# snap-research/MMVID

Measured on AMD Instinct MI355X. Metric: video-tokens/sec training step, 8-frame 128px text-to-video, higher is better.
Workload: dtype bf16

## Files before the change

### include/mmvid_hip_ext.h

```cpp
#ifndef MMVID_HIP_EXT_H
#define MMVID_HIP_EXT_H
#include <stdint.h>
#ifdef __cplusplus
extern "C" {
#endif

int mmvid_variates_fill(const int64_t* seeds, const int32_t* substream, int64_t videos, int64_t rows_per_video, int64_t n,
                        int purpose, int kind, const int32_t* draw_dev, int64_t draw_first, int64_t draws,
                        float* out, void* stream);

int mmvid_ema_update(float* ema, const float* p, int64_t n, float decay, int warmup, int step, const float* step_dev,
                     const uint8_t* row_flags, int64_t table_lo, int64_t table_rows, int rowlen, void* stream);

int mmvid_step_guard(const float* sqnorm, float grad_scale, float* step_dev, int32_t* guard_i, float* guard_f, void* stream);
int mmvid_adam_step_guarded(float* p, const float* g, float* m, float* v, void* shadow_bf16, int64_t n, float lr, const float* lr_dev,
                            float beta1, float beta2, float eps, float weight_decay, int step, const float* step_dev, float max_norm,
                            const float* sqnorm, float grad_scale, const uint8_t* row_flags, int64_t table_lo, int64_t table_rows,
                            int rowlen, const int32_t* skip_dev, void* stream);
int mmvid_ema_update_guarded(float* ema, const float* p, int64_t n, float decay, int warmup, int step, const float* step_dev,
                             const uint8_t* row_flags, int64_t table_lo, int64_t table_rows, int rowlen, const int32_t* skip_dev,
                             void* stream);

int mmvid_logits_truncate_rows(const float* logits, const float* logits_u, int64_t ld, const float* scale_dev, int64_t rows_per_scale,
                               float logit_div, int top_k, float top_p, const int32_t* top_k_dev, const float* top_p_dev,
// ... 6 lines not shown
                        const uint8_t* row_flags, int64_t table_lo, int64_t table_rows, int rowlen, const int32_t* skip_dev,
                        int32_t every, int32_t slots, int32_t* count_dev, float* partials_f, int32_t* partials_i,
                        float* ring_f, int32_t* ring_i, int32_t* head_i, float* head_f, void* stream);

int mmvid_adam_step_decoupled(float* p, const float* g, float* m, float* v, void* shadow_bf16, int64_t n, float lr, const float* lr_dev,
                              float beta1, float beta2, float eps, float weight_decay, int step, const float* step_dev, float max_norm,
                              const float* sqnorm, float grad_scale, const uint8_t* row_flags, int64_t table_lo, int64_t table_rows,
                              int rowlen, const int32_t* skip_dev, void* stream);

int mmvid_lr_schedule_ext(const float* step_dev, int kind, float lr_min, float lr_max, int every, int64_t a, int64_t b, float gamma,
                          float* lr_out, void* stream);

int mmvid_lr_plateau(const float* loss_dev, const float* step_dev, int every, float factor, int patience, int cooldown, float threshold,
                     float min_lr, float eps, float* state_f, int32_t* state_i, const int32_t* skip_dev, void* stream);

#ifdef __cplusplus
}
#endif
#endif
```

### mmvid_amd/clip_tower.py

```python
import ctypes
import os
import math

import torch
from torch import nn

from . import _lib, ops
from .functional import _note_params, _with_param_zeros
from .shadow import Bf16Weight

TOWER_SHAPES = {
    'openai_clip_visual': (768, 12, 12),
    'openai_clip_text': (512, 12, 8),
}
MAX_WIDTH = 1024
MATRIX_KEYS = ('attn.in_proj_weight', 'attn.out_proj.weight', 'mlp.c_fc.weight', 'mlp.c_proj.weight')


def check_tower_width(width, source):
    if width <= 0 or width % 64:
        raise ValueError(f'{source}: tower width {width} is not a multiple of 64 (the attention kernels take heads of 64: heads = width / 64)')
    if width > MAX_WIDTH:
        raise ValueError(f'{source}: tower width {width} is above {MAX_WIDTH}, the widest tower the kernels take '
                         '(ViT-L/14 visual towers are 1024 wide; ViT-H and larger are not supported)')
# ... 53 lines not shown
        self.resblocks = nn.ModuleList([ResidualAttentionBlockParams(width, layers) for _ in range(layers)])


class _TowerFn(torch.autograd.Function):
    @staticmethod
    def forward(ctx, x, tower, keep, *params):
        _note_params(ctx, (x, tower, keep) + params)
        ctx.tower = tower
        y, saved = tower._run_forward(x, keep=keep)
        ctx.saved_arena = saved
        ctx.shape = x.shape
        return y

    @staticmethod
    def backward(ctx, gy):
        g = gy.contiguous().clone()
        ctx.tower._run_backward(g, ctx.saved_arena, ctx.shape)
        ctx.saved_arena = None
        return _with_param_zeros(ctx, (g.view(ctx.shape), None, None) + (None, ) * (len(ctx.needs_input_grad) - 3))


class DecodeSession:

    def __init__(self, tower, kv_cache, first_pos, graph, fused=True):
        self.tower, self.cache, self.fused = tower, kv_cache, fused
        B, dev = kv_cache.shape[1], kv_cache.device
        self.cfg = tower._cfg(B, kv_cache.shape[2])
        self.layers, self._keep = tower._layer_structs(False)
        _, self.scratch = tower._workspace(self.cfg, dev, False)
        self.x = torch.zeros(B, tower.width, device=dev, dtype=torch.float32)
        self.y = torch.zeros_like(self.x)
        self.pos = torch.tensor([first_pos], dtype=torch.int32, device=dev)
# ... 97 lines not shown
            raise ValueError(f'dim={model_dim} does not match the tower: {source} gives a {which_model} tower {width} wide; pass dim={width}')
        self.width, self.layers, self.heads = width or w, layers or l, heads or h
        self.debug_keep_saved = False
        assert self.width == 64 * self.heads, 'head_dim must be 64 (CLIP towers)'
        self.context_length = seq_len
        self.causal = causal
        self.transformer = _TowerParams(self.width, self.layers)
        self.mask_spec = self.build_attention_mask(seq_len, mask_type, **(mask_kwargs or {})) if causal else None
        if model_path is not None:
            self.load_clip_checkpoint(model_path, which_model, sd)
        self._matrix_holders = [h for blk in self.transformer.resblocks for h in (
            (blk.attn, 'in_proj_weight'), (blk.attn.out_proj, 'weight'), (blk.mlp.c_fc, 'weight'), (blk.mlp.c_proj, 'weight'))]
        self._bf16 = [None] * len(self._matrix_holders)
        self._scratch = None
        self._scratch_retired = []
        self.backward_chunk_layers = int(os.environ.get('MMVID_BWD_CHUNK', 0))
        self.on_layers_done = None

    @staticmethod
    def build_attention_mask(context_length, mask_type='causal', **kwargs):
        if mask_type == 'causal':
            return 'causal'
        if mask_type == 'mask_prev':
            idx = list(kwargs['index'])
            assert len(idx) <= 2, 'the kernels carry at most two restricted rows (BERT uses [ST1],[VID])'
            return ('rows', [(int(i), int(i)) for i in idx])
        raise NotImplementedError(mask_type)

    def dense_attention_mask(self, L=None):
        L = L or self.context_length
# ... 108 lines not shown
            a.g_out_w, a.g_out_b = gptr(blk.attn.out_proj.weight), gptr(blk.attn.out_proj.bias)
            a.g_fc_w, a.g_fc_b = gptr(blk.mlp.c_fc.weight), gptr(blk.mlp.c_fc.bias)
            a.g_pj_w, a.g_pj_b = gptr(blk.mlp.c_proj.weight), gptr(blk.mlp.c_proj.bias)
        return arr, keep

    def _workspace(self, cfg, device, keep):
        sb, cb = ctypes.c_int64(), ctypes.c_int64()
        _lib.call('mmvid_tower_workspace', ctypes.byref(cfg), ctypes.byref(sb), ctypes.byref(cb))
        if self._scratch is None or self._scratch.device != torch.device(device) or self._scratch.numel() < cb.value:
            if self._scratch is not None:
                self._scratch_retired.append(self._scratch)
            self._scratch = torch.empty(cb.value, device=device, dtype=torch.uint8)
        saved = torch.empty(sb.value, device=device, dtype=torch.uint8) if keep else None
        return saved, self._scratch

    def _run_forward(self, x, keep):
        x = ops._chk(x.contiguous(), torch.float32, 'tower input')
        B, L, _ = x.shape
        cfg = self._cfg(B, L)
        layers, _keep = self._layer_structs(False)
        saved, scratch = self._workspace(cfg, x.device, keep)
        y = torch.empty_like(x)
        _lib.call('mmvid_tower_forward', ctypes.byref(cfg), layers, ops._p(x), ops._p(y), ops._p(saved), ops._p(scratch),
                  ops._stream())
        if self.debug_keep_saved:
            self._last_saved = saved
        return y, saved

    def backward_chunks(self):
        if self.on_layers_done is None:
            return [(0, self.layers)]
        if self.backward_chunk_layers <= 0:
            return self._planned_chunks()
        step = self.backward_chunk_layers
        out, hi = [], self.layers
        while hi > 0:
# ... 4 lines not shown

    def _planned_chunks(self):
        if getattr(self, '_chunk_plan', None) is None or self._chunk_plan[0] != self.layers:
            E = self.width
            F = 4 * E
            t = sum(-(-n // 256) * -(-k // 128) for n, k in ((3 * E, E), (E, E), (F, E), (E, F)))
            waste = lambda n: (-(-n * t // 256)) - n * t / 256.0
            best, plan = None, [(0, self.layers)]
            for a in range(3, self.layers - 2):
                w = waste(a) + waste(self.layers - a) + 0.02 * abs(a - 0.6 * self.layers)
                if best is None or w < best:
                    best, plan = w, [(self.layers - a, self.layers), (0, self.layers - a)]
            self._chunk_plan = (self.layers, plan)
        return self._chunk_plan[1]

    def _run_backward(self, g, saved, shape):
        if saved is None:
            raise _lib.MMVIDError('tower backward without saved activations (forward ran under no_grad)')
        B, L, _ = shape
        cfg = self._cfg(B, L)
        layers, _keep = self._layer_structs(True)
        _, scratch = self._workspace(cfg, g.device, False)
        sb = ctypes.c_int64()
        _lib.call('mmvid_tower_workspace', ctypes.byref(cfg), ctypes.byref(sb), None)
        if sb.value != saved.numel():
            raise _lib.MMVIDError(f'tower backward: the saved arena holds {saved.numel()} bytes, the current layout needs {sb.value} '
                                  '(the library changed between forward and backward)')
        per_layer = saved.numel() // self.layers
        for lo, hi in self.backward_chunks():
            sub = self._cfg(B, L)
            sub.layers = hi - lo
            lp = ctypes.cast(ctypes.byref(layers, lo * ctypes.sizeof(_lib.TowerLayer)), ctypes.POINTER(_lib.TowerLayer))
            _lib.call('mmvid_tower_backward', ctypes.byref(sub), lp, ops._p(g),
                      ctypes.c_void_p(saved.data_ptr() + lo * per_layer), ops._p(scratch), ops._stream())
            if self.on_layers_done is not None:
                self.on_layers_done(lo)
```

### mmvid_amd/csrc/embed.hip

```cpp
#include "../../include/mmvid_hip.h"
#include "common.h"

namespace {

constexpr int MAX_TABLES = 4;
struct Tables {
    const float* t[MAX_TABLES];
    long rows[MAX_TABLES];
};
struct GradTables {
    float* t[MAX_TABLES];
    long rows[MAX_TABLES];
};

__device__ unsigned long long g_faults[4];

__global__ __launch_bounds__(256) void assemble_fwd_kernel(Tables tb, const long long* __restrict__ ids,
                                                           const int* __restrict__ seg,
                                                           const float* __restrict__ pos, long nrows, int L, int E,
                                                           float* __restrict__ out) {
    const long row = (long)blockIdx.x * 4 + (threadIdx.x >> 6);
    if (row >= nrows) return;
    const int lane = threadIdx.x & 63;
    const int l = (int)(row % L);
// ... 160 lines not shown
    const float l = lse[row];
    long t = target[row];
    if (t < 0 || t >= V) t = 0;
    const float4* p = reinterpret_cast<const float4*>(logits + row * ldl);
    for (int c = lane; c < (V >> 2); c += 64) {
        const float4 v = p[c];
        float o[4] = {__expf(v.x - l), __expf(v.y - l), __expf(v.z - l), __expf(v.w - l)};
        const long base = (long)c * 4;
#pragma unroll
        for (int e = 0; e < 4; ++e)
            if (base + e == t) o[e] -= 1.0f;
        d[c] = make_uint2(pack_bf2(o[0] * gs, o[1] * gs), pack_bf2(o[2] * gs, o[3] * gs));
    }
}

template <bool DET>
__global__ __launch_bounds__(256) void colsum_bf16_kernel(const bf16_t* __restrict__ dy, long ld, long M, int N,
                                                          float* __restrict__ db) {
    __shared__ float red[8][256];
    const int cc = threadIdx.x & 31, rg = threadIdx.x >> 5;
    const int n = (blockIdx.x * 32 + cc) * 8;
    const long m0 = (long)blockIdx.y * 256;
    float a[8];
#pragma unroll
    for (int e = 0; e < 8; ++e) a[e] = 0.f;
    if (n < N) {
        long m1 = m0 + 256;
        if (m1 > M) m1 = M;
        for (long m = m0 + rg; m < m1; m += 8) {
            const uint4 w = *reinterpret_cast<const uint4*>(dy + m * ld + n);
            a[0] += bf_lo(w.x), a[1] += bf_hi(w.x), a[2] += bf_lo(w.y), a[3] += bf_hi(w.y);
            a[4] += bf_lo(w.z), a[5] += bf_hi(w.z), a[6] += bf_lo(w.w), a[7] += bf_hi(w.w);
        }
    }
#pragma unroll
    for (int e = 0; e < 8; ++e) red[rg][cc * 8 + e] = a[e];
    __syncthreads();
    const int col = threadIdx.x;
    const int gn = blockIdx.x * 256 + col;
    if (gn < N) {
        float s = 0.f;
#pragma unroll
        for (int r = 0; r < 8; ++r) s += red[r][col];
        if (DET)
            db[(long)blockIdx.y * N + gn] = s;
        else
            unsafeAtomicAdd(db + gn, s);
    }
}
// ... 249 lines not shown
                                       const uint8_t* select, const float* lse, const float* gscale, int64_t rows,
                                       int V, void* dlogits_bf16, int64_t ldd, void* stream) {
    MMVID_REQUIRE(logits && target && lse && gscale && dlogits_bf16, "cross_entropy_bwd: null pointer");
    MMVID_REQUIRE(V % 4 == 0 && ldl % 4 == 0 && ldd % 4 == 0, "cross_entropy_bwd: V/ld must be multiples of 4");
    if (rows == 0) return MMVID_OK;
    hipLaunchKernelGGL(ce_bwd_kernel, dim3(cdiv(rows, 4)), dim3(256), 0, (hipStream_t)stream, logits, (long)ldl,
                       (const long long*)target, select, lse, gscale, (long)rows, V, (bf16_t*)dlogits_bf16, (long)ldd);
    MMVID_LAUNCH_CHECK("cross_entropy_bwd");
    return MMVID_OK;
}

extern "C" int mmvid_colsum_bf16(const void* dy, int64_t ld, int64_t M, int N, float* db, void* stream) {
    MMVID_REQUIRE(dy && db, "colsum_bf16: null pointer");
    MMVID_REQUIRE(N % 8 == 0 && ld % 8 == 0, "colsum_bf16: N and ld must be multiples of 8");
    if (M == 0) return MMVID_OK;
    hipLaunchKernelGGL(colsum_bf16_kernel<false>, dim3(cdiv(N, 256), cdiv(M, 256)), dim3(256), 0, (hipStream_t)stream,
                       (const bf16_t*)dy, (long)ld, (long)M, N, db);
    MMVID_LAUNCH_CHECK("colsum_bf16");
    return MMVID_OK;
}

int mmvid_slab_reduce(const float* slab, int nslabs, int N, float* out, hipStream_t stream) {
    hipLaunchKernelGGL(slab_reduce_kernel, dim3(cdiv(N, 32)), dim3(256), 0, stream, slab, nslabs, N, out);
    return MMVID_OK;
}

extern "C" int64_t mmvid_colsum_bf16_det_workspace_bytes(int64_t M, int N) { return (int64_t)cdiv(M > 0 ? M : 1, 256) * N * 4; }

extern "C" int mmvid_colsum_bf16_det(const void* dy, int64_t ld, int64_t M, int N, float* db, void* workspace,
                                     int64_t workspace_bytes, void* stream) {
    MMVID_REQUIRE(dy && db, "colsum_bf16_det: null pointer");
    MMVID_REQUIRE(N % 8 == 0 && ld % 8 == 0, "colsum_bf16_det: N and ld must be multiples of 8");
    if (M == 0) return MMVID_OK;
    MMVID_REQUIRE(workspace && workspace_bytes >= mmvid_colsum_bf16_det_workspace_bytes(M, N),
                  "colsum_bf16_det: workspace of %lld bytes needed (mmvid_colsum_bf16_det_workspace_bytes)",
                  (long long)mmvid_colsum_bf16_det_workspace_bytes(M, N));
    const int blocks = cdiv(M, 256);
    hipLaunchKernelGGL(colsum_bf16_kernel<true>, dim3(cdiv(N, 256), blocks), dim3(256), 0, (hipStream_t)stream, (const bf16_t*)dy,
                       (long)ld, (long)M, N, (float*)workspace);
    mmvid_slab_reduce((const float*)workspace, blocks, N, db, (hipStream_t)stream);
    MMVID_LAUNCH_CHECK("colsum_bf16_det");
    return MMVID_OK;
}

extern "C" int64_t mmvid_cross_entropy_fwd_det_workspace_bytes(int64_t rows) { return (rows > 0 ? rows : 1) * 4; }

extern "C" int mmvid_cross_entropy_fwd_det(const float* logits, int64_t ldl, const int64_t* target, const uint8_t* select,
                                           int64_t rows, int V, float* lse, float* loss_sum, void* workspace,
                                           int64_t workspace_bytes, void* stream) {
    MMVID_REQUIRE(logits && target && lse && loss_sum, "cross_entropy_fwd_det: null pointer");
    MMVID_REQUIRE(V % 4 == 0 && ldl % 4 == 0, "cross_entropy_fwd_det: V and ldl must be multiples of 4");
    if (rows == 0) return MMVID_OK;
    MMVID_REQUIRE(workspace && workspace_bytes >= rows * 4, "cross_entropy_fwd_det: workspace of %lld bytes needed", (long long)rows * 4);
    hipLaunchKernelGGL(ce_fwd_kernel<true>, dim3(cdiv(rows, 4)), dim3(256), 0, (hipStream_t)stream, logits, (long)ldl,
// ... 318 lines not shown
```

### mmvid_amd/csrc/tower.hip

```cpp
#include "../../include/mmvid_hip.h"
#include "common.h"
#include <vector>

#include "graphs.h"

namespace {

inline int64_t align256(int64_t x) { return (x + 255) & ~(int64_t)255; }
constexpr int kMaxSplitK = 16;
constexpr int kLnBwdBlocks = 512;

struct Dims {
    int B, L, E, H, F, layers;
    int64_t M;
};
Dims dims_of(const mmvid_tower_cfg_t& c) {
    Dims d;
    d.B = c.B, d.L = c.L, d.E = c.E, d.H = c.H, d.F = c.F, d.layers = c.layers;
    d.M = (int64_t)c.B * c.L;
    return d;
}

struct SavedLayer {
    int64_t x_in, x_mid, mean1, rstd1, mean2, rstd2, h1, qkv, o, lse2, h2, pre, act, k_gpj, k_dpre, k_gout, k_dqkv, k_ln1, k_ln2, total;
// ... 88 lines not shown
}

}

extern "C" int mmvid_tower_workspace(const mmvid_tower_cfg_t* cfg, int64_t* saved_bytes, int64_t* scratch_bytes) {
    TRY(check_cfg(cfg));
    const Dims d = dims_of(*cfg);
    if (saved_bytes) *saved_bytes = saved_layout(d).total * d.layers;
    if (scratch_bytes) *scratch_bytes = scratch_layout(d).total;
    return MMVID_OK;
}

static int tower_forward_enqueue(const mmvid_tower_cfg_t* cfg, const mmvid_tower_layer_t* layers, const float* x_in,
                                 float* x_out, void* saved, void* scratch, void* stream, void* kv_cache = nullptr,
                                 int kv_lmax = 0);
static int tower_backward_enqueue(const mmvid_tower_cfg_t* cfg, const mmvid_tower_layer_t* layers, float* g,
                                  void* saved, void* scratch, void* stream);

static uint64_t tower_key(uint64_t seed, const mmvid_tower_cfg_t* cfg, const mmvid_tower_layer_t* layers, const void* a,
                          const void* b, const void* c, const void* d, const void* stream) {
    uint64_t k = mmvid_hash_bytes(cfg, sizeof(*cfg), 0xcbf29ce484222325ull ^ seed);
    k = mmvid_hash_bytes(layers, sizeof(mmvid_tower_layer_t) * (size_t)cfg->layers, k);
    return mmvid_hash_ptr(stream, mmvid_hash_ptr(d, mmvid_hash_ptr(c, mmvid_hash_ptr(b, mmvid_hash_ptr(a, k)))));
}

extern "C" int mmvid_tower_forward(const mmvid_tower_cfg_t* cfg, const mmvid_tower_layer_t* layers,
                                   const float* x_in, float* x_out, void* saved, void* scratch, void* stream) {
    TRY(check_cfg(cfg));
    MMVID_REQUIRE(layers && x_in && x_out && scratch, "tower_forward: null pointer");
    const uint64_t key = tower_key(2, cfg, layers, x_in, x_out, saved, scratch, stream);
    return mmvid_run_cached(key, (hipStream_t)stream, [=](hipStream_t s) {
        return tower_forward_enqueue(cfg, layers, x_in, x_out, saved, scratch, (void*)s);
    });
}

static int tower_forward_enqueue(const mmvid_tower_cfg_t* cfg, const mmvid_tower_layer_t* layers, const float* x_in,
                                 float* x_out, void* saved, void* scratch, void* stream, void* kv_cache, int kv_lmax) {
    const Dims d = dims_of(*cfg);
    const SavedLayer sl = saved_layout(d);
    const Scratch sc = scratch_layout(d);
    char* scr = (char*)scratch;
    const float scale = 0.125f;
    const float* x = x_in;
    for (int i = 0; i < d.layers; ++i) {
        const mmvid_tower_layer_t& ly = layers[i];
        char* sv = saved ? (char*)saved + (int64_t)i * sl.total : scr + sc.infer;
        float* xin_s = (float*)(sv + sl.x_in);
        float* xmid = (float*)(sv + sl.x_mid);
        if (saved && i == 0) {
            if (hipMemcpyAsync(xin_s, x_in, d.M * d.E * 4, hipMemcpyDeviceToDevice, (hipStream_t)stream) != hipSuccess) {
                mmvid_set_error("tower_forward: memcpy failed");
                return MMVID_ERR_HIP;
            }
            x = xin_s;
        }
        float* xnext;
        if (i == d.layers - 1)
            xnext = x_out;
        else if (saved)
            xnext = (float*)((char*)saved + (int64_t)(i + 1) * sl.total + sl.x_in);
        else
            xnext = x_out;
        TRY(mmvid_layernorm_fwd(x, d.E, d.M, d.E, ly.ln1_w, ly.ln1_b, cfg->ln_eps, sv + sl.h1, nullptr, d.E,
                                (float*)(sv + sl.mean1), (float*)(sv + sl.rstd1), stream));
        TRY(linear_fwd(d.M, 3 * d.E, d.E, sv + sl.h1, ly.in_w, ly.in_b, nullptr, nullptr, 0, nullptr, sv + sl.qkv, stream));
        if (kv_cache)
            TRY(mmvid_kv_store(sv + sl.qkv, 3 * d.E, d.B, d.L, d.E, nullptr, 0, kv_lmax,
                               (char*)kv_cache + (int64_t)i * d.B * kv_lmax * 2 * d.E * 2, stream));
        TRY(mmvid_attention_fwd(sv + sl.qkv, 3 * d.E, d.B, d.L, d.H, d.E, scale, cfg->mask_mode, cfg->r0, cfg->c0, cfg->r1,
                                cfg->c1, sv + sl.o, d.E, (float*)(sv + sl.lse2), stream));
        TRY(linear_fwd(d.M, d.E, d.E, sv + sl.o, ly.out_w, ly.out_b, x, nullptr, 0, xmid, nullptr, stream));
        TRY(mmvid_layernorm_fwd(xmid, d.E, d.M, d.E, ly.ln2_w, ly.ln2_b, cfg->ln_eps, sv + sl.h2, nullptr, d.E,
                                (float*)(sv + sl.mean2), (float*)(sv + sl.rstd2), stream));
        TRY(linear_fwd(d.M, d.F, d.E, sv + sl.h2, ly.fc_w, ly.fc_b, nullptr, saved ? sv + sl.pre : nullptr, 1, nullptr,
                       sv + sl.act, stream));
        TRY(linear_fwd(d.M, d.E, d.F, sv + sl.act, ly.pj_w, ly.pj_b, xmid, nullptr, 0, xnext, nullptr, stream));
        x = xnext;
    }
    return MMVID_OK;
}

extern "C" int mmvid_tower_backward(const mmvid_tower_cfg_t* cfg, const mmvid_tower_layer_t* layers, float* g,
                                    void* saved, void* scratch, void* stream) {
    TRY(check_cfg(cfg));
    MMVID_REQUIRE(layers && g && saved && scratch, "tower_backward: null pointer");
    const uint64_t key = tower_key(mmvid_option(MMVID_OPT_DETERMINISTIC) ? 5 : 3, cfg, layers, g, saved, scratch, nullptr, stream);
    return mmvid_run_cached(key, (hipStream_t)stream, [=](hipStream_t s) {
        return tower_backward_enqueue(cfg, layers, g, saved, scratch, (void*)s);
    });
}

static int tower_backward_enqueue(const mmvid_tower_cfg_t* cfg, const mmvid_tower_layer_t* layers, float* g, void* saved,
                                  void* scratch, void* stream) {
    const Dims d = dims_of(*cfg);
    const SavedLayer sl = saved_layout(d);
    const Scratch sc = scratch_layout(d);
    char* scr = (char*)scratch;
    char* keep = (char*)saved;
    struct { int64_t g_pj, d_pre, g_out, dqkv, total; } kl = {sl.k_gpj, sl.k_dpre, sl.k_gout, sl.k_dqkv, sl.total};
    const float scale = 0.125f;
    void* d_h = scr + sc.d_h;
    float* ws = (float*)(scr + sc.splitk_ws);
    void* det_ws = nullptr;
    const int64_t det_bytes = det_slab_bytes(d);
    if (mmvid_option(MMVID_OPT_DETERMINISTIC)) {
        MMVID_REQUIRE(det_bytes <= sc.total - sc.infer, "tower_backward: the deterministic slabs do not fit the scratch arena");
        det_ws = scr + sc.infer;
    }
    const int64_t ln_ws_floats = (int64_t)kLnBwdBlocks * 3 * d.E;
    std::vector<mmvid_ln_reduce_t> ln_items;
    int ln_blocks = 0;
    for (int i = d.layers - 1; i >= 0; --i) {
        const mmvid_tower_layer_t& ly = layers[i];
        const char* sv = (const char*)saved + (int64_t)i * sl.total;
        char* kp = keep + (int64_t)i * kl.total;
        void* g_pj = kp + kl.g_pj;
        if (i == d.layers - 1) {
            TRY(mmvid_cast_f32_to_bf16(g, g_pj, d.M * d.E, stream));
            if (ly.g_pj_b && det_ws) TRY(mmvid_colsum_bf16_det(g_pj, d.E, d.M, d.E, ly.g_pj_b, det_ws, det_bytes, stream));
            if (ly.g_pj_b && !det_ws) TRY(mmvid_colsum_bf16(g_pj, d.E, d.M, d.E, ly.g_pj_b, stream));
        }
        TRY(linear_dx(d.M, d.E, d.F, g_pj, ly.pj_w, sv + sl.pre, nullptr, kp + kl.d_pre, stream, ly.g_fc_b, det_ws, det_bytes));
        TRY(linear_dx(d.M, d.F, d.E, kp + kl.d_pre, ly.fc_w, nullptr, nullptr, d_h, stream));
        {
            mmvid_ln_reduce_t r = {(const float*)(kp + sl.k_ln2), ly.g_ln2_w, ly.g_ln2_b, ly.g_out_b};
            int nb = 0;
            TRY(mmvid_layernorm_bwd_partial(d_h, 1, d.E, (const float*)(sv + sl.x_mid), d.E, (const float*)(sv + sl.mean2),
                                            (const float*)(sv + sl.rstd2), ly.ln2_w, d.M, d.E, g, d.E, 1, kp + kl.g_out, r.dw != nullptr,
                                            r.db != nullptr, r.dx_colsum != nullptr, (float*)(kp + sl.k_ln2), ln_ws_floats, &nb, stream));
            if (r.dw || r.db || r.dx_colsum) ln_items.push_back(r), ln_blocks = nb;
        }
        TRY(linear_dx(d.M, d.E, d.E, kp + kl.g_out, ly.out_w, nullptr, nullptr, scr + sc.d_o, stream));
        if (det_ws)
            TRY(mmvid_attention_bwd_bias_det(sv + sl.qkv, 3 * d.E, sv + sl.o, d.E, scr + sc.d_o, d.E, (const float*)(sv + sl.lse2),
                                             (float*)(scr + sc.delta), d.B, d.L, d.H, d.E, scale, cfg->mask_mode, cfg->r0, cfg->c0,
// ... 96 lines not shown
```

### mmvid_amd/dalle_artv.py

```python
import torch
import torch.nn.functional as F
from torch import nn

from . import artv_sampling, ops, sampling, seeded, token_draw
from .artv_sampling import k_keep, keep_top
from .clip_tower import OpenAICLIPTransformer, check_tower_width
from .dalle_bert import DivideMax, eval_decorator, exists, set_requires_grad
from .frontend import Frontend, check_condition_drop, face_choices
from .functional import AssembleSequence, LNLinear, LNLinearCrossEntropy
from .modules import AxialPositionalEmbedding, AxialPositionalEmbeddingList
from .shadow import Bf16Weight

NEG = -torch.finfo(torch.float32).max


def is_empty(t):
    return t.nelement() == 0


def top_k(logits, thres=0.5):
    return keep_top(logits, k_keep(thres, logits.shape[-1]))


class DALLE(nn.Module):
# ... 150 lines not shown
        return text, torch.where(vis_tok == -1, vis_pad, vis_tok)

    def _pos_rows(self):
        return torch.cat([self.text_pos_emb.weight, self.visual_pos_emb.table(), self.image_pos_emb.table()], 0)

    def _hidden(self, text, vis_tok, image):
        text, visual = self._prompt_ids(text, vis_tok)
        parts = [text, visual]
        if exists(image) and not is_empty(image):
            image = self.get_image_tokens(image)
            parts.append(image)
        ids = torch.cat(parts, 1)
        if ids.shape[1] > self.total_seq_len:
            ids = ids[:, :-1]
        L = ids.shape[1]
        x = AssembleSequence.apply(self._pos_rows()[:L], ids.contiguous(), self._seg[:L].contiguous(), self.text_emb.weight,
                                   self.visual_emb.weight, self.image_emb.weight)
        out = self.transformer(x)
        if self.stable:
            out = self.norm_by_max(out)
        return out, text, visual, image

    def _logits_rows(self, rows, cols=None):
        lin = self.to_logits[1]
        if cols is None:
            return LNLinear.apply(rows, self.to_logits[0].weight, self.to_logits[0].bias, lin.weight, lin.bias, self._w16())
        with torch.no_grad():
            hn = ops.layernorm_fwd(rows.contiguous(), self.to_logits[0].weight, self.to_logits[0].bias, 1e-5, save_stats=False)[0]
            return ops.gemm(hn, self._w16()[cols[0]:cols[1]], bias=lin.bias.detach()[cols[0]:cols[1]], out_dtype=torch.float32)

    def forward(self, text, visual=None, target=None, return_loss=False, erase_visual=False, erase_visual_half=False,
# ... 176 lines not shown
```

### mmvid_amd/dalle_bert.py

```python
import torch
import torch.nn.functional as F
from torch import nn

from . import ops, sampling, seeded
from .clip_tower import OpenAICLIPTransformer, check_tower_width
from .frontend import Frontend, check_condition_drop, face_choices
from .functional import PosTable, AssembleSequence, BertHeads, LNLinear, Linear, LayerNormRows
from .shadow import Bf16Weight
from .modules import AxialPositionalEmbedding, AxialPositionalEmbeddingList


def exists(val):
    return val is not None


def set_requires_grad(model, value):
    if model is not None:
        for p in model.parameters():
            p.requires_grad = value


def eval_decorator(fn):
    def inner(model, *args, **kwargs):
        was_training = model.training
# ... 274 lines not shown
        choices, frame0 = face_choices(vc_mode, face_mode)
        return self.frontend.erase_choice(image, tv, f, self.image_token_lut['[MASK]'], choices, frame0)

    def _visual_tokens(self, visual, erase_visual, erase_visual_half, vc_mode, face_mode, visual_aug_mode):
        if self.num_visuals == 0 or not (exists(visual) and len(visual)):
            return None
        if visual_aug_mode == 'motion_color' and torch.is_tensor(visual) and visual.dim() == 5:
            visual = self.frontend.visual_color_jitter(visual, 0.9, 1)
        tok = self.get_image_tokens(visual, insert_sep=self.insert_sep, which_vae='cvae')
        if erase_visual:
            tok = self.random_erase_codebook(tok, self.visual_eraser, erase_visual_half)
        if vc_mode is not None:
            tok = self.erase_codebook_face(tok, vc_mode, face_mode)
        return tok

    def _assemble(self, ids, length, text_rows=None):
        pos = self._pos_table()[:length]
        x = AssembleSequence.apply(pos, ids.contiguous(), self._seg[:length].contiguous(), *self._tables())
        if x.requires_grad:
            x.register_hook(self._note_table_backward)
        if text_rows is not None:
            x[:, self.txt_tok_index].add_(text_rows)
        return x

    def _map_text_feature(self, feat):
        m = self.text_feature_mapping
        if isinstance(m, nn.Linear):
            return Linear.apply(feat, m.weight, m.bias, self._w16(m))
        h = LNLinear.apply(feat, m[0].weight, m[0].bias, m[1].weight, m[1].bias, self._w16(m[1]))
        h = LNLinear.apply(h, m[2].weight, m[2].bias, m[3].weight, m[3].bias, self._w16(m[3]))
        return LayerNormRows.apply(h, m[4].weight, m[4].bias)

    def _head_rows(self, B, nseq, device):
# ... 102 lines not shown
        self.frontend.advance(device)

        if rel:
            assert B >= 2 and B % 2 == 0
        text_neg_ids = None
        if rel and negvc:
            text_neg_ids = ops._chk(text_neg.contiguous(), torch.int64, 'text_neg')
        ids, sel, tfull, cnt = ops.bert_build_ids(text, vis_tok, self.visual_seq_len, target, target_warp, mask1, pad_base, MASK,
                                                  bool(rel), bool(do_vid), text_neg=text_neg_ids)
        self._log_text_ids(ids)
        if text_rows is not None and (rel or do_vid):
            half = B // 2
            per_pass = [text_rows] + ([torch.cat((text_rows[half:], text_rows[:half]))] if rel else []) + \
                ([text_rows] if do_vid else [])
            text_rows = torch.cat(per_pass)
        x_seq = self._assemble(ids, self.total_seq_len, text_rows)
        if text_neg_ids is not None and self.num_visuals > 0 and self.visual_seq_len > 0:
            L = self.total_seq_len
            v0 = 1 + self.text_seq_len
            keep = torch.cat((torch.arange(0, v0, device=device), torch.arange(v0 + self.visual_seq_len, L, device=device)))
            x_neg = x_seq[B:2 * B].index_select(1, keep).contiguous()
            x_main = torch.cat((x_seq[:B], x_seq[2 * B:])) if do_vid else x_seq[:B]
            y_main = self.transformer_forward(x_main.contiguous())
            y_neg = self.transformer_forward(x_neg)
            y_rel = torch.zeros(B, L, y_neg.shape[-1], device=device, dtype=y_neg.dtype).index_copy(1, keep, y_neg)
            y = torch.cat((y_main[:B], y_rel, y_main[B:])) if do_vid else torch.cat((y_main, y_rel))
        else:
            y = self.transformer_forward(x_seq)
        if self._debug_keep is not None:
            self._debug_keep.update(mask1=mask1, nfm=not_fully_masked, target=target, target_warp=target_warp, ids=ids, sel=sel,
                                    tfull=tfull, cnt=cnt, x_seq=x_seq, y=y)
        nseq = 1 + int(bool(rel)) + int(bool(do_vid))
# ... 66 lines not shown
```

### mmvid_amd/functional.py

```python
import torch

from . import ops

bf16, f32 = torch.bfloat16, torch.float32


def _grad_buf(p):
    if p.grad is None:
        p.grad = torch.zeros_like(p)
    return p.grad


_ZERO = {}


def _inside_ddp():
    ddp = getattr(torch.nn.parallel, 'DistributedDataParallel', None)
    return ddp is not None and getattr(ddp, '_active_ddp_module', None) is not None


def _note_params(ctx, args):
    ctx._ddp_params = [a if (isinstance(a, torch.nn.Parameter) and a.requires_grad) else None for a in args] if _inside_ddp() else None


# ... 3 lines not shown
        return grads
    out = list(grads)
    for i, p in enumerate(ps):
        if p is not None and i < len(out) and out[i] is None:
            _grad_buf(p)
            key = (p.device, p.dtype)
            if key not in _ZERO:
                _ZERO[key] = torch.zeros((), device=p.device, dtype=p.dtype)
            out[i] = _ZERO[key].expand(p.shape)
    return tuple(out)


class AssembleSequence(torch.autograd.Function):

    @staticmethod
    def forward(ctx, pos, ids, seg, *tables):
        _note_params(ctx, (pos, ids, seg) + tables)
        ctx.tables = tables
        ctx.save_for_backward(ids, seg)
        return ops.assemble_sequence([t.detach() for t in tables], ids, seg, pos.detach().contiguous())

    @staticmethod
    def backward(ctx, dx):
        ids, seg = ctx.saved_tensors
        dx = dx.contiguous()
        gts = [_grad_buf(t) if t.requires_grad else None for t in ctx.tables]
        dpos = torch.empty(dx.shape[1:], device=dx.device, dtype=f32) if ctx.needs_input_grad[0] else None
        ops.assemble_sequence_bwd(gts, [t.shape[0] for t in ctx.tables], ids, seg, dx, dpos)
        return _with_param_zeros(ctx, (dpos, None, None) + (None, ) * len(ctx.tables))


class PosTable(torch.autograd.Function):

    @staticmethod
    def forward(ctx, layout, L, *params):
        from . import _lib
        _note_params(ctx, (layout, L) + params)
        E = params[0].shape[-1]
        ctx.layout, ctx.L, ctx.E = layout, L, E
        out = torch.empty(L, E, device=params[0].device, dtype=f32)
        segs = PosTable._segments(layout, grads=False)
        _lib.call('mmvid_pos_table_fwd', segs, len(layout), L, E, ops._p(out), ops._stream())
        return out

# ... 220 lines not shown
```

### mmvid_amd/ops.py

```python
import ctypes

import torch

from . import _lib
from ._lib import call

bf16, f32, i64 = torch.bfloat16, torch.float32, torch.int64


def _stream():
    return ctypes.c_void_p(torch.cuda.current_stream().cuda_stream)


def _p(t):
    if t is None:
        return None
    return ctypes.c_void_p(t.data_ptr())


def capture_graph(fn):
    g, side = torch.cuda.CUDAGraph(), torch.cuda.Stream()
    side.wait_stream(torch.cuda.current_stream())
    with torch.cuda.stream(side), torch.cuda.graph(g, stream=side):
        fn()
# ... 303 lines not shown
    if dbias is not None and _lib.is_deterministic():
        ws = _det_ws('attention_bwd_bias', qkv.device, _lib.load().mmvid_attention_bwd_bias_det_workspace_bytes(B, L, E))
        call('mmvid_attention_bwd_bias_det', _p(qkv), 3 * E, _p(out), E, _p(dout), E, _p(lse2), _p(delta), B, L, H, E, float(scale),
             *_mask_args(mask), _p(dqkv), 3 * E, _p(dbias), _p(ws), ws.numel(), _stream())
        return dqkv
    call('mmvid_attention_bwd_bias', _p(qkv), 3 * E, _p(out), E, _p(dout), E, _p(lse2), _p(delta), B, L, H, E, float(scale),
         *_mask_args(mask), _p(dqkv), 3 * E, _p(dbias) if dbias is not None else None, _stream())
    return dqkv


def _ptr_array(tensors):
    arr = (ctypes.c_void_p * len(tensors))(*[t.data_ptr() if t is not None else 0 for t in tensors])
    return ctypes.cast(arr, ctypes.POINTER(ctypes.c_void_p)), arr


def assemble_sequence(tables, ids, seg, pos):
    B, L = ids.shape
    E = pos.shape[-1]
    for t in tables:
        _chk(t, f32, 'table')
    _chk(ids, i64, 'ids'), _chk(pos, f32, 'pos')
    assert seg.dtype == torch.int32 and seg.is_cuda
    out = torch.empty(B, L, E, device=ids.device, dtype=f32)
    tp, keep = _ptr_array(tables)
    rows = (ctypes.c_int64 * len(tables))(*[t.shape[0] for t in tables])
    call('mmvid_assemble_sequence', tp, rows, len(tables), _p(ids), _p(seg), _p(pos), B, L, E, _p(out), _stream())
    return out


def assemble_sequence_bwd(grad_tables, table_rows, ids, seg, dx, dpos=None, accumulate_dpos=False):
    B, L = ids.shape
    E = dx.shape[-1]
    _chk(dx, f32, 'dx')
    tp, keep = _ptr_array(grad_tables)
    rows = (ctypes.c_int64 * len(grad_tables))(*table_rows)
    if _lib.is_deterministic():
        nb = _lib.load().mmvid_assemble_sequence_bwd_det_workspace_bytes(B, L, E, len(grad_tables), rows)
        if nb < 0:
# ... 529 lines not shown
```

Baseline: 214,200.

## Write tower input in place and fuse backward grad entry copy, cast and bias colsum

The sequence assembly now writes its output straight into the tower's saved-activation slot, so the forward pass skips the device-to-device copy of the input. In backward, the clone of the incoming gradient plus the separate f32-to-bf16 cast and bias column sum are merged into one kernel. That kernel reads gy once and writes the f32 copy, the bf16 copy and the colsum together. This cuts several full-activation memory passes per step, at the cost of more coupling between the embedding, autograd in-place marking and the tower workspace lifetime.

New measurement: 214,800 (median of 5 runs). About the same (+0.3%).

```diff
diff --git a/include/mmvid_hip_ext.h b/include/mmvid_hip_ext.h
--- a/include/mmvid_hip_ext.h
+++ b/include/mmvid_hip_ext.h
@@ -44,6 +44,10 @@
 int mmvid_lr_plateau(const float* loss_dev, const float* step_dev, int every, float factor, int patience, int cooldown, float threshold,
                      float min_lr, float eps, float* state_f, int32_t* state_i, const int32_t* skip_dev, void* stream);
 
+int mmvid_tower_saved_x_in(const void* cfg, int64_t* offset_bytes);
+int mmvid_grad_entry_bf16(const float* gy, int64_t M, int N, float* g, void* g_bf16, float* db, void* stream);
+int mmvid_tower_backward_from(const void* cfg, const void* layers, const float* gy, float* g, void* saved, void* scratch, void* stream);
+
 #ifdef __cplusplus
 }
 #endif
diff --git a/mmvid_amd/clip_tower.py b/mmvid_amd/clip_tower.py
--- a/mmvid_amd/clip_tower.py
+++ b/mmvid_amd/clip_tower.py
@@ -91,8 +91,9 @@
 
     @staticmethod
     def backward(ctx, gy):
-        g = gy.contiguous().clone()
-        ctx.tower._run_backward(g, ctx.saved_arena, ctx.shape)
+        gy = gy.contiguous()
+        g = torch.empty_like(gy)
+        ctx.tower._run_backward(gy, g, ctx.saved_arena, ctx.shape)
         ctx.saved_arena = None
         return _with_param_zeros(ctx, (g.view(ctx.shape), None, None) + (None, ) * (len(ctx.needs_input_grad) - 3))
 
@@ -220,6 +221,7 @@
         self._bf16 = [None] * len(self._matrix_holders)
         self._scratch = None
         self._scratch_retired = []
+        self._slot_ahead = None
         self.backward_chunk_layers = int(os.environ.get('MMVID_BWD_CHUNK', 0))
         self.on_layers_done = None
 
@@ -358,12 +360,27 @@
         saved = torch.empty(sb.value, device=device, dtype=torch.uint8) if keep else None
         return saved, self._scratch
 
+    def input_slot(self, B, L, device, x_requires_grad):
+        if not (torch.is_grad_enabled() and (x_requires_grad or self._any_trainable())):
+            return None
+        cfg = self._cfg(B, L)
+        saved, _ = self._workspace(cfg, device, True)
+        off = ctypes.c_int64()
+        _lib.call('mmvid_tower_saved_x_in', ctypes.byref(cfg), ctypes.byref(off))
+        x = torch.empty(0, device=device, dtype=torch.float32).set_(saved.untyped_storage(), (saved.storage_offset() + off.value) // 4,
+                                                                    (B, L, self.width))
+        self._slot_ahead = (saved, x.data_ptr(), (B, L))
+        return x
+
     def _run_forward(self, x, keep):
         x = ops._chk(x.contiguous(), torch.float32, 'tower input')
         B, L, _ = x.shape
         cfg = self._cfg(B, L)
         layers, _keep = self._layer_structs(False)
-        saved, scratch = self._workspace(cfg, x.device, keep)
+        ahead, self._slot_ahead = self._slot_ahead, None
+        saved, scratch = self._workspace(cfg, x.device, keep and not (ahead and ahead[1:] == (x.data_ptr(), (B, L))))
+        if keep and saved is None:
+            saved = ahead[0]
         y = torch.empty_like(x)
         _lib.call('mmvid_tower_forward', ctypes.byref(cfg), layers, ops._p(x), ops._p(y), ops._p(saved), ops._p(scratch),
                   ops._stream())
@@ -398,7 +415,7 @@
             self._chunk_plan = (self.layers, plan)
         return self._chunk_plan[1]
 
-    def _run_backward(self, g, saved, shape):
+    def _run_backward(self, gy, g, saved, shape):
         if saved is None:
             raise _lib.MMVIDError('tower backward without saved activations (forward ran under no_grad)')
         B, L, _ = shape
@@ -415,7 +432,7 @@
             sub = self._cfg(B, L)
             sub.layers = hi - lo
             lp = ctypes.cast(ctypes.byref(layers, lo * ctypes.sizeof(_lib.TowerLayer)), ctypes.POINTER(_lib.TowerLayer))
-            _lib.call('mmvid_tower_backward', ctypes.byref(sub), lp, ops._p(g),
+            _lib.call('mmvid_tower_backward_from', ctypes.byref(sub), lp, ops._p(gy if hi == self.layers else g), ops._p(g),
                       ctypes.c_void_p(saved.data_ptr() + lo * per_layer), ops._p(scratch), ops._stream())
             if self.on_layers_done is not None:
                 self.on_layers_done(lo)
diff --git a/mmvid_amd/csrc/embed.hip b/mmvid_amd/csrc/embed.hip
--- a/mmvid_amd/csrc/embed.hip
+++ b/mmvid_amd/csrc/embed.hip
@@ -1,4 +1,5 @@
 #include "../../include/mmvid_hip.h"
+#include "../../include/mmvid_hip_ext.h"
 #include "common.h"
 
 namespace {
@@ -198,25 +199,67 @@
     }
 }
 
-template <bool DET>
-__global__ __launch_bounds__(256) void colsum_bf16_kernel(const bf16_t* __restrict__ dy, long ld, long M, int N,
-                                                          float* __restrict__ db) {
+struct ColsumBf16Rows {
+    static constexpr int ROWS = 256, UNROLL = 1;
+    static constexpr bool SUMS_OPTIONAL = false;
+    const bf16_t* dy;
+    long ld;
+    typedef uint4 Row;
+    __device__ __forceinline__ Row load(long m, int n) const { return *reinterpret_cast<const uint4*>(dy + m * ld + n); }
+    __device__ __forceinline__ uint4 row8(const Row& r, long, int) const { return r; }
+};
+struct GradEntryRows {
+    static constexpr int ROWS = 64, UNROLL = 4;
+    static constexpr bool SUMS_OPTIONAL = true;
+    const float* gy;
+    float* g;
+    bf16_t* g16;
+    long ld;
+    struct Row {
+        float4 v0, v1;
+    };
+    __device__ __forceinline__ Row load(long m, int n) const {
+        const float4* src = reinterpret_cast<const float4*>(gy + m * ld + n);
+        return Row{src[0], src[1]};
+    }
+    __device__ __forceinline__ uint4 row8(const Row& r, long m, int n) const {
+        const float4 v0 = r.v0, v1 = r.v1;
+        const uint4 w = make_uint4(pack_bf2(v0.x, v0.y), pack_bf2(v0.z, v0.w), pack_bf2(v1.x, v1.y), pack_bf2(v1.z, v1.w));
+        *reinterpret_cast<uint4*>(g16 + m * ld + n) = w;
+        if (g != gy) {
+            float4* dst = reinterpret_cast<float4*>(g + m * ld + n);
+            dst[0] = v0, dst[1] = v1;
+        }
+        return w;
+    }
+};
+template <bool DET, typename SRC>
+__global__ __launch_bounds__(256) void colsum_bf16_kernel(const SRC src, long M, int N, float* __restrict__ db) {
     __shared__ float red[8][256];
     const int cc = threadIdx.x & 31, rg = threadIdx.x >> 5;
     const int n = (blockIdx.x * 32 + cc) * 8;
-    const long m0 = (long)blockIdx.y * 256;
+    const long m0 = (long)blockIdx.y * SRC::ROWS;
     float a[8];
 #pragma unroll
     for (int e = 0; e < 8; ++e) a[e] = 0.f;
     if (n < N) {
-        long m1 = m0 + 256;
+        long m1 = m0 + SRC::ROWS;
         if (m1 > M) m1 = M;
-        for (long m = m0 + rg; m < m1; m += 8) {
-            const uint4 w = *reinterpret_cast<const uint4*>(dy + m * ld + n);
-            a[0] += bf_lo(w.x), a[1] += bf_hi(w.x), a[2] += bf_lo(w.y), a[3] += bf_hi(w.y);
-            a[4] += bf_lo(w.z), a[5] += bf_hi(w.z), a[6] += bf_lo(w.w), a[7] += bf_hi(w.w);
-        }
-    }
+        for (long m = m0 + rg; m < m1; m += 8 * SRC::UNROLL) {
+            typename SRC::Row r[SRC::UNROLL];
+#pragma unroll
+            for (int u = 0; u < SRC::UNROLL; ++u)
+                if (SRC::UNROLL == 1 || m + 8 * u < m1) r[u] = src.load(m + 8 * u, n);
+#pragma unroll
+            for (int u = 0; u < SRC::UNROLL; ++u)
+                if (SRC::UNROLL == 1 || m + 8 * u < m1) {
+                    const uint4 w = src.row8(r[u], m + 8 * u, n);
+                    a[0] += bf_lo(w.x), a[1] += bf_hi(w.x), a[2] += bf_lo(w.y), a[3] += bf_hi(w.y);
+                    a[4] += bf_lo(w.z), a[5] += bf_hi(w.z), a[6] += bf_lo(w.w), a[7] += bf_hi(w.w);
+                }
+        }
+    }
+    if (SRC::SUMS_OPTIONAL && !db) return;
 #pragma unroll
     for (int e = 0; e < 8; ++e) red[rg][cc * 8 + e] = a[e];
     __syncthreads();
@@ -496,9 +539,22 @@
     MMVID_REQUIRE(dy && db, "colsum_bf16: null pointer");
     MMVID_REQUIRE(N % 8 == 0 && ld % 8 == 0, "colsum_bf16: N and ld must be multiples of 8");
     if (M == 0) return MMVID_OK;
-    hipLaunchKernelGGL(colsum_bf16_kernel<false>, dim3(cdiv(N, 256), cdiv(M, 256)), dim3(256), 0, (hipStream_t)stream,
-                       (const bf16_t*)dy, (long)ld, (long)M, N, db);
+    hipLaunchKernelGGL((colsum_bf16_kernel<false, ColsumBf16Rows>), dim3(cdiv(N, 256), cdiv(M, ColsumBf16Rows::ROWS)), dim3(256), 0,
+                       (hipStream_t)stream, ColsumBf16Rows{(const bf16_t*)dy, (long)ld}, (long)M, N, db);
     MMVID_LAUNCH_CHECK("colsum_bf16");
+    return MMVID_OK;
+}
+
+extern "C" int mmvid_grad_entry_bf16(const float* gy, int64_t M, int N, float* g, void* g_bf16, float* db, void* stream) {
+    MMVID_REQUIRE(gy && g && g_bf16, "grad_entry_bf16: null pointer");
+    MMVID_REQUIRE(N > 0 && N % 8 == 0 && M >= 0 && cdiv(M, GradEntryRows::ROWS) <= 65535,
+                  "grad_entry_bf16: N must be a multiple of 8 and M at most 65535 * %d rows", GradEntryRows::ROWS);
+    MMVID_REQUIRE(((uintptr_t)gy & 15) == 0 && ((uintptr_t)g & 15) == 0 && ((uintptr_t)g_bf16 & 15) == 0,
+                  "grad_entry_bf16: buffers must be 16-byte aligned");
+    if (M == 0) return MMVID_OK;
+    hipLaunchKernelGGL((colsum_bf16_kernel<false, GradEntryRows>), dim3(cdiv(N, 256), cdiv(M, GradEntryRows::ROWS)), dim3(256), 0,
+                       (hipStream_t)stream, GradEntryRows{gy, g, (bf16_t*)g_bf16, (long)N}, (long)M, N, db);
+    MMVID_LAUNCH_CHECK("grad_entry_bf16");
     return MMVID_OK;
 }
 
@@ -518,8 +574,8 @@
                   "colsum_bf16_det: workspace of %lld bytes needed (mmvid_colsum_bf16_det_workspace_bytes)",
                   (long long)mmvid_colsum_bf16_det_workspace_bytes(M, N));
     const int blocks = cdiv(M, 256);
-    hipLaunchKernelGGL(colsum_bf16_kernel<true>, dim3(cdiv(N, 256), blocks), dim3(256), 0, (hipStream_t)stream, (const bf16_t*)dy,
-                       (long)ld, (long)M, N, (float*)workspace);
+    hipLaunchKernelGGL((colsum_bf16_kernel<true, ColsumBf16Rows>), dim3(cdiv(N, 256), blocks), dim3(256), 0, (hipStream_t)stream,
+                       ColsumBf16Rows{(const bf16_t*)dy, (long)ld}, (long)M, N, (float*)workspace);
     mmvid_slab_reduce((const float*)workspace, blocks, N, db, (hipStream_t)stream);
     MMVID_LAUNCH_CHECK("colsum_bf16_det");
     return MMVID_OK;
diff --git a/mmvid_amd/csrc/tower.hip b/mmvid_amd/csrc/tower.hip
--- a/mmvid_amd/csrc/tower.hip
+++ b/mmvid_amd/csrc/tower.hip
@@ -1,4 +1,5 @@
 #include "../../include/mmvid_hip.h"
+#include "../../include/mmvid_hip_ext.h"
 #include "common.h"
 #include <vector>
 
@@ -126,7 +127,7 @@
 static int tower_forward_enqueue(const mmvid_tower_cfg_t* cfg, const mmvid_tower_layer_t* layers, const float* x_in,
                                  float* x_out, void* saved, void* scratch, void* stream, void* kv_cache = nullptr,
                                  int kv_lmax = 0);
-static int tower_backward_enqueue(const mmvid_tower_cfg_t* cfg, const mmvid_tower_layer_t* layers, float* g,
+static int tower_backward_enqueue(const mmvid_tower_cfg_t* cfg, const mmvid_tower_layer_t* layers, const float* gy, float* g,
                                   void* saved, void* scratch, void* stream);
 
 static uint64_t tower_key(uint64_t seed, const mmvid_tower_cfg_t* cfg, const mmvid_tower_layer_t* layers, const void* a,
@@ -134,6 +135,14 @@
     uint64_t k = mmvid_hash_bytes(cfg, sizeof(*cfg), 0xcbf29ce484222325ull ^ seed);
     k = mmvid_hash_bytes(layers, sizeof(mmvid_tower_layer_t) * (size_t)cfg->layers, k);
     return mmvid_hash_ptr(stream, mmvid_hash_ptr(d, mmvid_hash_ptr(c, mmvid_hash_ptr(b, mmvid_hash_ptr(a, k)))));
+}
+
+extern "C" int mmvid_tower_saved_x_in(const void* cfg_, int64_t* offset_bytes) {
+    const mmvid_tower_cfg_t* cfg = (const mmvid_tower_cfg_t*)cfg_;
+    TRY(check_cfg(cfg));
+    MMVID_REQUIRE(offset_bytes, "tower_saved_x_in: null pointer");
+    *offset_bytes = saved_layout(dims_of(*cfg)).x_in;
+    return MMVID_OK;
 }
 
 extern "C" int mmvid_tower_forward(const mmvid_tower_cfg_t* cfg, const mmvid_tower_layer_t* layers,
@@ -159,13 +168,13 @@
         char* sv = saved ? (char*)saved + (int64_t)i * sl.total : scr + sc.infer;
         float* xin_s = (float*)(sv + sl.x_in);
         float* xmid = (float*)(sv + sl.x_mid);
-        if (saved && i == 0) {
+        if (saved && i == 0 && x_in != xin_s) {
             if (hipMemcpyAsync(xin_s, x_in, d.M * d.E * 4, hipMemcpyDeviceToDevice, (hipStream_t)stream) != hipSuccess) {
                 mmvid_set_error("tower_forward: memcpy failed");
                 return MMVID_ERR_HIP;
             }
-            x = xin_s;
         }
+        if (saved && i == 0) x = xin_s;
         float* xnext;
         if (i == d.layers - 1)
             xnext = x_out;
@@ -192,18 +201,25 @@
     return MMVID_OK;
 }
 
+extern "C" int mmvid_tower_backward_from(const void* cfg_, const void* layers_, const float* gy, float* g, void* saved, void* scratch,
+                                         void* stream) {
+    const mmvid_tower_cfg_t* cfg = (const mmvid_tower_cfg_t*)cfg_;
+    const mmvid_tower_layer_t* layers = (const mmvid_tower_layer_t*)layers_;
+    TRY(check_cfg(cfg));
+    MMVID_REQUIRE(layers && gy && g && saved && scratch, "tower_backward: null pointer");
+    const uint64_t key = tower_key(mmvid_option(MMVID_OPT_DETERMINISTIC) ? 5 : 3, cfg, layers, g, saved, scratch, gy, stream);
+    return mmvid_run_cached(key, (hipStream_t)stream, [=](hipStream_t s) {
+        return tower_backward_enqueue(cfg, layers, gy, g, saved, scratch, (void*)s);
+    });
+}
+
 extern "C" int mmvid_tower_backward(const mmvid_tower_cfg_t* cfg, const mmvid_tower_layer_t* layers, float* g,
                                     void* saved, void* scratch, void* stream) {
-    TRY(check_cfg(cfg));
-    MMVID_REQUIRE(layers && g && saved && scratch, "tower_backward: null pointer");
-    const uint64_t key = tower_key(mmvid_option(MMVID_OPT_DETERMINISTIC) ? 5 : 3, cfg, layers, g, saved, scratch, nullptr, stream);
-    return mmvid_run_cached(key, (hipStream_t)stream, [=](hipStream_t s) {
-        return tower_backward_enqueue(cfg, layers, g, saved, scratch, (void*)s);
-    });
-}
-
-static int tower_backward_enqueue(const mmvid_tower_cfg_t* cfg, const mmvid_tower_layer_t* layers, float* g, void* saved,
-                                  void* scratch, void* stream) {
+    return mmvid_tower_backward_from(cfg, layers, g, g, saved, scratch, stream);
+}
+
+static int tower_backward_enqueue(const mmvid_tower_cfg_t* cfg, const mmvid_tower_layer_t* layers, const float* gy, float* g,
+                                  void* saved, void* scratch, void* stream) {
     const Dims d = dims_of(*cfg);
     const SavedLayer sl = saved_layout(d);
     const Scratch sc = scratch_layout(d);
@@ -228,9 +244,8 @@
         char* kp = keep + (int64_t)i * kl.total;
         void* g_pj = kp + kl.g_pj;
         if (i == d.layers - 1) {
-            TRY(mmvid_cast_f32_to_bf16(g, g_pj, d.M * d.E, stream));
+            TRY(mmvid_grad_entry_bf16(gy, d.M, d.E, g, g_pj, det_ws ? nullptr : ly.g_pj_b, stream));
             if (ly.g_pj_b && det_ws) TRY(mmvid_colsum_bf16_det(g_pj, d.E, d.M, d.E, ly.g_pj_b, det_ws, det_bytes, stream));
-            if (ly.g_pj_b && !det_ws) TRY(mmvid_colsum_bf16(g_pj, d.E, d.M, d.E, ly.g_pj_b, stream));
         }
         TRY(linear_dx(d.M, d.E, d.F, g_pj, ly.pj_w, sv + sl.pre, nullptr, kp + kl.d_pre, stream, ly.g_fc_b, det_ws, det_bytes));
         TRY(linear_dx(d.M, d.F, d.E, kp + kl.d_pre, ly.fc_w, nullptr, nullptr, d_h, stream));
diff --git a/mmvid_amd/dalle_artv.py b/mmvid_amd/dalle_artv.py
--- a/mmvid_amd/dalle_artv.py
+++ b/mmvid_amd/dalle_artv.py
@@ -188,7 +188,7 @@
         if ids.shape[1] > self.total_seq_len:
             ids = ids[:, :-1]
         L = ids.shape[1]
-        x = AssembleSequence.apply(self._pos_rows()[:L], ids.contiguous(), self._seg[:L].contiguous(), self.text_emb.weight,
+        x = AssembleSequence.apply(self._pos_rows()[:L], ids.contiguous(), self._seg[:L].contiguous(), None, self.text_emb.weight,
                                    self.visual_emb.weight, self.image_emb.weight)
         out = self.transformer(x)
         if self.stable:
diff --git a/mmvid_amd/dalle_bert.py b/mmvid_amd/dalle_bert.py
--- a/mmvid_amd/dalle_bert.py
+++ b/mmvid_amd/dalle_bert.py
@@ -312,9 +312,13 @@
             tok = self.erase_codebook_face(tok, vc_mode, face_mode)
         return tok
 
-    def _assemble(self, ids, length, text_rows=None):
+    def _assemble(self, ids, length, text_rows=None, for_tower=False):
         pos = self._pos_table()[:length]
-        x = AssembleSequence.apply(pos, ids.contiguous(), self._seg[:length].contiguous(), *self._tables())
+        tables = self._tables()
+        out = None
+        if for_tower:
+            out = self.transformer.input_slot(ids.shape[0], length, ids.device, pos.requires_grad or any(t.requires_grad for t in tables))
+        x = AssembleSequence.apply(pos, ids.contiguous(), self._seg[:length].contiguous(), out, *tables)
         if x.requires_grad:
             x.register_hook(self._note_table_backward)
         if text_rows is not None:
@@ -447,8 +451,9 @@
             per_pass = [text_rows] + ([torch.cat((text_rows[half:], text_rows[:half]))] if rel else []) + \
                 ([text_rows] if do_vid else [])
             text_rows = torch.cat(per_pass)
-        x_seq = self._assemble(ids, self.total_seq_len, text_rows)
-        if text_neg_ids is not None and self.num_visuals > 0 and self.visual_seq_len > 0:
+        split_neg = text_neg_ids is not None and self.num_visuals > 0 and self.visual_seq_len > 0
+        x_seq = self._assemble(ids, self.total_seq_len, text_rows, for_tower=not split_neg)
+        if split_neg:
             L = self.total_seq_len
             v0 = 1 + self.text_seq_len
             keep = torch.cat((torch.arange(0, v0, device=device), torch.arange(v0 + self.visual_seq_len, L, device=device)))
diff --git a/mmvid_amd/functional.py b/mmvid_amd/functional.py
--- a/mmvid_amd/functional.py
+++ b/mmvid_amd/functional.py
@@ -41,11 +41,13 @@
 class AssembleSequence(torch.autograd.Function):
 
     @staticmethod
-    def forward(ctx, pos, ids, seg, *tables):
-        _note_params(ctx, (pos, ids, seg) + tables)
+    def forward(ctx, pos, ids, seg, out, *tables):
+        _note_params(ctx, (pos, ids, seg, out) + tables)
         ctx.tables = tables
         ctx.save_for_backward(ids, seg)
-        return ops.assemble_sequence([t.detach() for t in tables], ids, seg, pos.detach().contiguous())
+        if out is not None:
+            ctx.mark_dirty(out)
+        return ops.assemble_sequence([t.detach() for t in tables], ids, seg, pos.detach().contiguous(), out=out)
 
     @staticmethod
     def backward(ctx, dx):
@@ -54,7 +56,7 @@
         gts = [_grad_buf(t) if t.requires_grad else None for t in ctx.tables]
         dpos = torch.empty(dx.shape[1:], device=dx.device, dtype=f32) if ctx.needs_input_grad[0] else None
         ops.assemble_sequence_bwd(gts, [t.shape[0] for t in ctx.tables], ids, seg, dx, dpos)
-        return _with_param_zeros(ctx, (dpos, None, None) + (None, ) * len(ctx.tables))
+        return _with_param_zeros(ctx, (dpos, None, None, None) + (None, ) * len(ctx.tables))
 
 
 class PosTable(torch.autograd.Function):
diff --git a/mmvid_amd/ops.py b/mmvid_amd/ops.py
--- a/mmvid_amd/ops.py
+++ b/mmvid_amd/ops.py
@@ -341,14 +341,16 @@
     return ctypes.cast(arr, ctypes.POINTER(ctypes.c_void_p)), arr
 
 
-def assemble_sequence(tables, ids, seg, pos):
+def assemble_sequence(tables, ids, seg, pos, out=None):
     B, L = ids.shape
     E = pos.shape[-1]
     for t in tables:
         _chk(t, f32, 'table')
     _chk(ids, i64, 'ids'), _chk(pos, f32, 'pos')
     assert seg.dtype == torch.int32 and seg.is_cuda
-    out = torch.empty(B, L, E, device=ids.device, dtype=f32)
+    if out is None:
+        out = torch.empty(B, L, E, device=ids.device, dtype=f32)
+    assert _chk(out, f32, 'out').shape == (B, L, E)
     tp, keep = _ptr_array(tables)
     rows = (ctypes.c_int64 * len(tables))(*[t.shape[0] for t in tables])
     call('mmvid_assemble_sequence', tp, rows, len(tables), _p(ids), _p(seg), _p(pos), B, L, E, _p(out), _stream())
```
